# stsievert/pytorch-ps-mpi

Measured on AMD Instinct MI355X. Metric: samples/sec (node) ResNet-50 async PS at 1/2/4/8 MI355X; grad bytes/step, higher is better.
Workload: dtype bf16

## Files before the change

hipps/csrc/bindings.cpp:

```cpp
#include <torch/extension.h>
#include <vector>

namespace hipps {
void aggregate(const std::vector<at::Tensor>& slots, at::Tensor acc, double gscale, bool accumulate, bool acquire);
void copy_acquire(at::Tensor src, at::Tensor dst);
void convert(at::Tensor src, at::Tensor dst, double scale);
void gather_flat(const std::vector<at::Tensor>& srcs, at::Tensor table, at::Tensor dst, double scale);
void transpose_cast(at::Tensor src, at::Tensor dst, at::Tensor tiles);
void sgd_step(const std::vector<at::Tensor>& grads, double gscale, at::Tensor p, c10::optional<at::Tensor> buf,
              c10::optional<at::Tensor> pub, bool zero_src, double lr, double wd, double momentum, double dampening,
              bool nesterov, bool first, c10::optional<at::Tensor> mask, c10::optional<at::Tensor> csteps,
              double lookahead);
void adam_step(const std::vector<at::Tensor>& grads, double gscale, at::Tensor p, at::Tensor exp_avg,
               at::Tensor exp_avg_sq, c10::optional<at::Tensor> max_exp_avg_sq, c10::optional<at::Tensor> pub,
               bool zero_src, double lr, double beta1, double beta2, double eps, double wd, int64_t step,
               bool amsgrad, bool torch_mode, c10::optional<at::Tensor> mask, c10::optional<at::Tensor> csteps);
void q8_encode(at::Tensor x, c10::optional<at::Tensor> resid, at::Tensor q, at::Tensor scales, bool stochastic,
               int64_t seed);
void q8_aggregate(const std::vector<at::Tensor>& qs, const std::vector<at::Tensor>& ss, at::Tensor acc, double gscale,
                  bool accumulate, bool acquire);
void topk_encode(at::Tensor g, c10::optional<at::Tensor> resid, int64_t k, at::Tensor idx, at::Tensor val,
                 at::Tensor workspace);
int64_t topk_workspace_bytes(int64_t n, int64_t k);
void topk_accumulate(at::Tensor idx, at::Tensor val, at::Tensor acc, double gscale, bool acquire);
// ... 23 lines not shown
void bn_backward_partials(at::Tensor part, int64_t nrb, at::Tensor dy, at::Tensor x, int64_t mask_mode,
                          at::Tensor weight, at::Tensor mean, at::Tensor invstd, at::Tensor scale, at::Tensor shift,
                          at::Tensor dx, c10::optional<at::Tensor> dres, at::Tensor dweight, at::Tensor dbias, int64_t C,
                          c10::optional<at::Tensor> mask_in, int64_t unr);
int64_t conv1x1_mtiles(int64_t M);
void conv1x1_forward(at::Tensor x, at::Tensor w, at::Tensor y, c10::optional<at::Tensor> part, int64_t Hi,
                     int64_t Wi, int64_t stride, c10::optional<at::Tensor> add, c10::optional<at::Tensor> add_mask,
                     c10::optional<at::Tensor> bn_x, c10::optional<at::Tensor> bn_bits,
                     c10::optional<at::Tensor> bn_mean, c10::optional<at::Tensor> bn_invstd,
                     c10::optional<at::Tensor> bn_scale, c10::optional<at::Tensor> bn_shift,
                     c10::optional<at::Tensor> pro_scale, c10::optional<at::Tensor> pro_shift);
void bn_dual_forward(at::Tensor part3, int64_t nrb3, at::Tensor partd, int64_t nrbd, at::Tensor x3, at::Tensor xd,
                     at::Tensor z, at::Tensor mask, at::Tensor w3, at::Tensor b3, at::Tensor rm3, at::Tensor rv3,
                     at::Tensor mean3, at::Tensor invstd3, at::Tensor scale3, at::Tensor shift3, at::Tensor wd,
                     at::Tensor bd, at::Tensor rmd, at::Tensor rvd, at::Tensor meand, at::Tensor invstdd,
                     at::Tensor scaled, at::Tensor shiftd, int64_t C, double eps3, double mom3, double epsd,
                     double momd);
void bn_dual_backward(c10::optional<at::Tensor> part3, int64_t nrb3, at::Tensor dz, at::Tensor x3, at::Tensor xd,
                      at::Tensor mask, at::Tensor w3, at::Tensor mean3, at::Tensor invstd3, at::Tensor wd,
                      at::Tensor meand, at::Tensor invstdd, at::Tensor dx3, at::Tensor dxd, at::Tensor dw3,
                      at::Tensor db3, at::Tensor dwd, at::Tensor dbd, int64_t C, int64_t unr);
at::Tensor gemm2_dgrad_s2(at::Tensor dy, at::Tensor wf, at::Tensor dx, int64_t bm, int64_t bn,
                          c10::optional<at::Tensor> bn_x, c10::optional<at::Tensor> bn_bits,
                          c10::optional<at::Tensor> bn_mean, c10::optional<at::Tensor> bn_invstd,
                          c10::optional<at::Tensor> bn_scale, c10::optional<at::Tensor> bn_shift);
int64_t gemm2_mtiles(int64_t M, int64_t N, int64_t K, int64_t bm);
void gemm2_conv(at::Tensor x, at::Tensor w, at::Tensor y, c10::optional<at::Tensor> part,
                c10::optional<at::Tensor> add, c10::optional<at::Tensor> add_mask, int64_t Hi, int64_t Wi,
                int64_t stride, int64_t KH, int64_t KW, int64_t pad, int64_t bm, int64_t bn,
                c10::optional<at::Tensor> bn_x, c10::optional<at::Tensor> bn_bits, c10::optional<at::Tensor> bn_mean,
                c10::optional<at::Tensor> bn_invstd, c10::optional<at::Tensor> bn_scale,
                c10::optional<at::Tensor> bn_shift, int64_t stages, bool add_s2,
                c10::optional<at::Tensor> pro_scale, c10::optional<at::Tensor> pro_shift,
                c10::optional<at::Tensor> bias, c10::optional<at::Tensor> gelu_pre, int64_t gelu);
void gemm2_wgrad(at::Tensor dy, at::Tensor x, at::Tensor dw, int64_t KH, int64_t KW, int64_t stride, int64_t pad,
                 int64_t Hi, int64_t Wi, int64_t cfg, int64_t stages,
                 c10::optional<at::Tensor> pro_scale, c10::optional<at::Tensor> pro_shift, int64_t sdiv);
void maxpool3s2_forward(at::Tensor x, at::Tensor y, at::Tensor code, c10::optional<at::Tensor> scale,
                        c10::optional<at::Tensor> shift);
void bn_finalize_partials(at::Tensor part, int64_t nrb, int64_t M, at::Tensor weight, at::Tensor bias,
                          c10::optional<at::Tensor> running_mean, c10::optional<at::Tensor> running_var,
                          at::Tensor mean, at::Tensor invstd, at::Tensor scale, at::Tensor shift, int64_t C, double eps,
                          double momentum);
void maxpool3s2_backward(at::Tensor dy, at::Tensor code, at::Tensor dx);
std::vector<at::Tensor> xent_forward(at::Tensor logits, at::Tensor labels, int64_t ignore_index);
void colsum_fold(at::Tensor part, at::Tensor out);
void colsum_bf16(at::Tensor x, at::Tensor out);
std::vector<at::Tensor> attn_forward(at::Tensor q, at::Tensor k, at::Tensor v, bool causal, double scale,
                                     c10::optional<at::Tensor> kvlen);
std::vector<at::Tensor> attn_backward(at::Tensor dout, at::Tensor q, at::Tensor k, at::Tensor v, at::Tensor o,
                                      at::Tensor lse, bool causal, double scale, c10::optional<at::Tensor> kvlen,
                                      c10::optional<at::Tensor> dq_out, c10::optional<at::Tensor> dk_out,
                                      c10::optional<at::Tensor> dv_out);
void swiglu_forward(at::Tensor a, at::Tensor b, at::Tensor c);
void ln_forward(at::Tensor x, at::Tensor w, at::Tensor b, at::Tensor y, at::Tensor mean, at::Tensor rstd, double eps);
void ln_backward(at::Tensor dy, at::Tensor x, at::Tensor mean, at::Tensor rstd, at::Tensor w, at::Tensor dx,
                 at::Tensor dw, at::Tensor db, c10::optional<at::Tensor> dxsum);
void embed_forward(at::Tensor ids, c10::optional<at::Tensor> tt, at::Tensor word, at::Tensor pos, at::Tensor typ,
                   at::Tensor out);
void embed_pos_backward(at::Tensor dout, at::Tensor dpos, int64_t B, int64_t S);
void embed_seg_backward(at::Tensor dout, at::Tensor sid, at::Tensor perm, at::Tensor dtab);
void rms_forward(at::Tensor x, at::Tensor w, at::Tensor y, at::Tensor rstd, double eps, c10::optional<at::Tensor> add,
                 c10::optional<at::Tensor> xsum);
void rms_backward(at::Tensor dy, at::Tensor x, at::Tensor rstd, at::Tensor w, at::Tensor dx, at::Tensor dw,
                  c10::optional<at::Tensor> dres, c10::optional<at::Tensor> dx16);
void swiglu_backward(at::Tensor g, at::Tensor a, at::Tensor b, at::Tensor da, at::Tensor db);
void rope_apply(at::Tensor x, at::Tensor y, at::Tensor cs, at::Tensor sn, int64_t S, int64_t hd, double sign);
// ... 74 lines not shown
        py::arg("acc"), py::arg("gscale"), py::arg("acquire") = false);
  m.def("topk_q8_accumulate", &hipps::topk_q8_accumulate, "acc[idx] += gscale * deq(q)", py::arg("idx"), py::arg("q"),
        py::arg("scales"), py::arg("acc"), py::arg("gscale"), py::arg("acquire") = false);
  m.def("topk_q8_residual", &hipps::topk_q8_residual, "EF: r[idx] += v - deq(q)");
  m.def("thresh_encode", &hipps::thresh_encode, "variable-size |x|>tau sparsification, device count header");
  m.def("thresh_accumulate", &hipps::thresh_accumulate, "acc[idx[:count]] += gscale * val[:count]", py::arg("count"),
        py::arg("idx"), py::arg("val"), py::arg("acc"), py::arg("gscale"), py::arg("acquire") = false);
  m.def("copy_counted", &hipps::copy_counted, "copy a [count | idx | val] message moving only count entries");
  m.def("bn_forward_train", &hipps::bn_forward_train, "fused channels-last BN train fwd (+res) (+relu)");
  m.def("bn_apply", &hipps::bn_apply, "y = act(x*scale + shift (+res))");
  m.def("bn_backward", &hipps::bn_backward, "fused BN bwd with relu-mask recompute (+dres)");
  m.def("bn_forward_partials", &hipps::bn_forward_partials, "BN fwd finalize+apply from producer-reduced partials");
  m.def("bn_backward_partials", &hipps::bn_backward_partials, "BN bwd finalize+apply from consumer-reduced partials",
        py::arg("part"), py::arg("nrb"), py::arg("dy"), py::arg("x"), py::arg("mask_mode"), py::arg("weight"),
        py::arg("mean"), py::arg("invstd"), py::arg("scale"), py::arg("shift"), py::arg("dx"), py::arg("dres"),
        py::arg("dweight"), py::arg("dbias"), py::arg("C"), py::arg("mask_in"), py::arg("unr") = 0);
  m.def("conv1x1_mtiles", &hipps::conv1x1_mtiles);
  m.def("bn_dual_forward", &hipps::bn_dual_forward,
        "z = relu(bn3(x3) + bnd(xd)) from producer partials: two finalizes + one apply (downsample block)");
  m.def("bn_dual_backward", &hipps::bn_dual_backward,
        "backward of bn_dual_forward: dx3 + the downsample BN's reduction in one pass, then dxd",
        py::arg("part3"), py::arg("nrb3"), py::arg("dz"), py::arg("x3"), py::arg("xd"), py::arg("mask"), py::arg("w3"),
        py::arg("mean3"), py::arg("invstd3"), py::arg("wd"), py::arg("meand"), py::arg("invstdd"), py::arg("dx3"),
        py::arg("dxd"), py::arg("dw3"), py::arg("db3"), py::arg("dwd"), py::arg("dbd"), py::arg("C"),
        py::arg("unr") = 4);
  m.def("gemm2_mtiles", &hipps::gemm2_mtiles, py::arg("M"), py::arg("N"), py::arg("K"), py::arg("bm") = 0);
  m.def("gemm2_conv", &hipps::gemm2_conv, "second-generation MFMA conv GEMM (LDS-DMA staged, 256-row tiles)",
        py::arg("x"), py::arg("w"), py::arg("y"), py::arg("part") = py::none(), py::arg("add") = py::none(),
        py::arg("add_mask") = py::none(), py::arg("Hi"), py::arg("Wi"), py::arg("stride") = 1, py::arg("KH") = 1,
        py::arg("KW") = 1, py::arg("pad") = 0, py::arg("bm") = 0, py::arg("bn") = 0, py::arg("bn_x") = py::none(),
        py::arg("bn_bits") = py::none(), py::arg("bn_mean") = py::none(), py::arg("bn_invstd") = py::none(),
        py::arg("bn_scale") = py::none(), py::arg("bn_shift") = py::none(), py::arg("stages") = 2,
        py::arg("add_s2") = false, py::arg("pro_scale") = py::none(), py::arg("pro_shift") = py::none(),
        py::arg("bias") = py::none(), py::arg("gelu_pre") = py::none(), py::arg("gelu") = 0);
  m.def("gemm2_dgrad_s2", &hipps::gemm2_dgrad_s2,
        "stride-2 3x3 input gradient as four output-parity implicit GEMMs (+ BN-backward reduction)",
        py::arg("dy"), py::arg("wf"), py::arg("dx"), py::arg("bm") = 128, py::arg("bn") = 128,
        py::arg("bn_x") = py::none(), py::arg("bn_bits") = py::none(), py::arg("bn_mean") = py::none(),
        py::arg("bn_invstd") = py::none(), py::arg("bn_scale") = py::none(), py::arg("bn_shift") = py::none());
  m.def("gemm2_wgrad", &hipps::gemm2_wgrad, "conv weight gradient on the LDS-DMA MFMA core (split-M slabs)",
        py::arg("dy"), py::arg("x"), py::arg("dw"), py::arg("KH"), py::arg("KW"), py::arg("stride"), py::arg("pad"),
        py::arg("Hi"), py::arg("Wi"), py::arg("cfg") = 0, py::arg("stages") = 2, py::arg("pro_scale") = py::none(),
        py::arg("pro_shift") = py::none(), py::arg("sdiv") = 1);
  m.def("conv1x1_forward", &hipps::conv1x1_forward,
        "MFMA 1x1 conv (NHWC GEMM) with fused BN-stats epilogue and optional (+ add * mask) epilogue",
        pybind11::arg("x"), pybind11::arg("w"), pybind11::arg("y"), pybind11::arg("part"), pybind11::arg("Hi"),
        pybind11::arg("Wi"), pybind11::arg("stride"), pybind11::arg("add") = pybind11::none(),
        pybind11::arg("add_mask") = pybind11::none(), pybind11::arg("bn_x") = pybind11::none(),
        pybind11::arg("bn_bits") = pybind11::none(), pybind11::arg("bn_mean") = pybind11::none(),
        pybind11::arg("bn_invstd") = pybind11::none(), pybind11::arg("bn_scale") = pybind11::none(),
        pybind11::arg("bn_shift") = pybind11::none(), pybind11::arg("pro_scale") = pybind11::none(),
        pybind11::arg("pro_shift") = pybind11::none());
  m.def("convkxk_forward", &hipps::convkxk_forward,
        "MFMA KxK conv forward (implicit GEMM, channels-last bf16) with optional BN-statistics epilogue",
        pybind11::arg("x"), pybind11::arg("w"), pybind11::arg("y"), pybind11::arg("part") = pybind11::none(),
        pybind11::arg("stride") = 1, pybind11::arg("pad") = 1);
  m.def("stem_mtiles", &hipps::stem_mtiles, "number of BN partial-statistic columns of stem_forward");
  m.def("stem_forward", &hipps::stem_forward,
        "ResNet stem 7x7/s2/p3 3->64 conv forward on MFMA (channels-last bf16), optional BN-statistics epilogue",
        pybind11::arg("x"), pybind11::arg("w"), pybind11::arg("y"), pybind11::arg("part") = pybind11::none());
  m.def("stem_bnpool_backward", &hipps::stem_bnpool_backward,
        "backward of maxpool(relu(bn(stem(x)))): BN parameter grads + stem weight grad, no pool gradient "
        "materialised (the BN input gradient only with materialize_dy)",
        py::arg("dp"), py::arg("code"), py::arg("y"), py::arg("x"), py::arg("bn_weight"), py::arg("mean"),
        py::arg("invstd"), py::arg("scale"), py::arg("shift"), py::arg("dbn_w"), py::arg("dbn_b"), py::arg("dw"),
        py::arg("materialize_dy") = false, py::arg("quad") = true);
  m.def("stem_wgrad", &hipps::stem_wgrad, "ResNet stem 7x7/s2/p3 weight gradient on MFMA (fp32 dW, deterministic)");
// ... 82 lines not shown
```

hipps/csrc/gemm2.hip:

```cpp
#include "common.h"

#include <ATen/ATen.h>
#include <cstdlib>
#include <mutex>
#include <c10/hip/HIPStream.h>
#include <torch/extension.h>

namespace hipps {
namespace g2 {

typedef short bf16x8 __attribute__((ext_vector_type(8)));
typedef float f32x4 __attribute__((ext_vector_type(4)));
typedef float f32x16 __attribute__((ext_vector_type(16)));
typedef uint32_t u32x4 __attribute__((ext_vector_type(4)));
typedef __attribute__((address_space(3))) void lds_void;
typedef __attribute__((address_space(1))) void glb_void;

constexpr int BK = 64;

__device__ __attribute__((aligned(64))) const uint16_t kZero16[32] = {0};
__device__ __attribute__((aligned(64))) const uint8_t kOnes8[64] = {
    0xff, 0xff, 0xff, 0xff, 0xff, 0xff, 0xff, 0xff, 0xff, 0xff, 0xff, 0xff, 0xff, 0xff, 0xff, 0xff,
    0xff, 0xff, 0xff, 0xff, 0xff, 0xff, 0xff, 0xff, 0xff, 0xff, 0xff, 0xff, 0xff, 0xff, 0xff, 0xff,
    0xff, 0xff, 0xff, 0xff, 0xff, 0xff, 0xff, 0xff, 0xff, 0xff, 0xff, 0xff, 0xff, 0xff, 0xff, 0xff,
// ... 48 lines not shown
  const uint16_t* R;
  const uint8_t* RM;
  const uint16_t* bx;
  const uint8_t* bbits;
  const float *bmean, *binvstd, *bscale, *bshift;
  int M, N, K, Ho, Wo, Hi, Wi, stride, mtiles, ntiles;
  int KW, pad, Cin;
  int ldb;
  int pstride, pcol0;
  int ph, pw, Hx, Wx;
  int tdr[4], tdc[4], tko[4];
  const float *psc, *psh;
  const float* bias;
  uint16_t* Y2;
  int epf;
};

__device__ __forceinline__ uint32_t add_bf16x2(uint32_t a, uint32_t b) {
  return pack_bf16x2(__uint_as_float(a << 16) + __uint_as_float(b << 16),
                     __uint_as_float(a & 0xffff0000u) + __uint_as_float(b & 0xffff0000u));
}

__device__ __forceinline__ void glds16(const void* src, void* dst) {
  __builtin_amdgcn_global_load_lds((glb_void*)src, (lds_void*)dst, 16, 0, 0);
}

constexpr int waitcnt_vm(int n) { return (n & 15) | ((n >> 4) << 14) | (7 << 4) | (15 << 8); }
constexpr int waitcnt_lgkm(int n) { return 15 | (3 << 14) | (7 << 4) | ((n & 15) << 8); }

__host__ __device__ constexpr int khalf_swz(int row) {
  return ((0x1320 >> (4 * ((row >> 2) & 3))) & 3);
}

template <int BM, int BN, int EPI, bool TAPS, int NS>
__global__ __launch_bounds__((nthreads<BM, BN>())) void k_gemm(Args g) {
  constexpr int TM = Cfg<BM, BN>::TM, TN = Cfg<BM, BN>::TN;
  constexpr int WM = BM / TM, WN = BN / TN, NW = WM * WN, NT = 64 * NW;
  constexpr int FM = TM / 16, FN = TN / 16;
  constexpr bool KH = NS == 4;
  constexpr bool PP = NS == 5;
  constexpr bool M32 = NS == 6;
  constexpr int NSX = M32 ? 2 : NS;
  constexpr bool PAR = (EPI & kPar) != 0;
  constexpr bool PRO = (EPI & kPro) != 0;
  static_assert(!PAR || TAPS, "kPar needs the implicit-GEMM loader");
  static_assert(!PRO || NS == 2, "kPro: 2 LDS stages");
  static_assert(!PP || (BM == 256 && BN == 256), "ping-pong: 256x256 on 8 waves");
  static_assert(!M32 || (BM == 256 && BN == 256 && !PRO), "32x32x16 MFMA: the 256x256 tile");
  auto orow = [&](int m) -> int64_t {
    if constexpr (PAR) {
      const int hw = g.Ho * g.Wo;
      const int img = m / hw, rem = m - img * hw;
      const int a = rem / g.Wo, b = rem - a * g.Wo;
      return ((int64_t)img * g.Hx + 2 * a + g.ph) * g.Wx + 2 * b + g.pw;
    } else {
      return m;
    }
  };
  constexpr int STAGE = (BM + BN) * BK;
  constexpr int UNIT = (BM + BN) * 32;
  constexpr int RPI = KH ? 16 : 8;
  constexpr int AI = BM / RPI / NW;
  constexpr int BI = BN / RPI / NW;
  constexpr int EP = BN + 8;
  constexpr int NSB = (KH || PP || M32) ? 2 : NS;
  constexpr int SCR = (NSB * STAGE * 2 > BM * EP * 2 ? NSB * STAGE * 2 : BM * EP * 2);
  static_assert(AI >= 1 && BI >= 1, "tile too small for the wave count");
  static_assert(NS >= 2 && NS <= 6, "stages");
  constexpr int NG = AI + BI;
  constexpr int BIP = PP ? 2 * BI : BI;
  __shared__ __attribute__((aligned(16))) uint16_t lds[lds_bytes<BM, BN, NS>() / 2];

  const int nwg = gridDim.x, orig = blockIdx.x, xcd = orig & 7, q8 = nwg >> 3, r8 = nwg & 7;
  const int bid = (xcd < r8 ? xcd * (q8 + 1) : r8 * (q8 + 1) + (xcd - r8) * q8) + (orig >> 3);
  const int mt = bid / g.ntiles, nt = bid - mt * g.ntiles;
  const int m0 = mt * BM, n0 = nt * BN;
  const int t = threadIdx.x, lane = t & 63;
  const int w = __builtin_amdgcn_readfirstlane(t >> 6);
  const int wm = w / WN, wn = w - (w / WN) * WN;
  auto arb = [&](int i) { return PP ? (BM / 2) * wm + RPI * (i * (NW / 2) + wn) : RPI * (i * NW + w); };
  auto brb = [&](int i) { return PP ? RPI * (i * (NW / 2) + wn) : RPI * (i * NW + w); };
  const int lr = KH ? lane >> 2 : lane >> 3;
  const int lc = KH ? (lane & 3) ^ khalf_swz(lr)
                    : M32 ? (lane & 7) ^ (((lr >> 1) | ((w & 1) << 2)) & 7) : (lane & 7) ^ lr;

  const uint16_t* a_src[AI];
  int a_h[TAPS ? AI : 1], a_w[TAPS ? AI : 1];
  bool a_ok[AI];
#pragma unroll
  for (int i = 0; i < AI; ++i) {
    const int row = arb(i) + lr;
    int m = m0 + row;
    a_ok[i] = m < g.M;
    m = a_ok[i] ? m : g.M - 1;
    if constexpr (TAPS) {
      const int hw = g.Ho * g.Wo;
      const int img = m / hw, rem = m - img * hw;
      const int ho = rem / g.Wo, wo = rem - ho * g.Wo;
      a_h[i] = PAR ? ho : ho * g.stride - g.pad;
      a_w[i] = PAR ? wo : wo * g.stride - g.pad;
      a_src[i] = g.X + (int64_t)img * g.Hi * g.Wi * g.Cin + lc * 8;
    } else {
      int64_t src = m;
      if (g.stride != 1) {
        const int hw = g.Ho * g.Wo;
        const int img = m / hw, rem = m - img * hw;
        const int ho = rem / g.Wo, wo = rem - ho * g.Wo;
        src = ((int64_t)img * g.Hi + (int64_t)ho * g.stride) * g.Wi + (int64_t)wo * g.stride;
      }
      a_src[i] = g.X + src * g.K + lc * 8;
    }
  }
  const uint16_t* b_src0 = g.W + (int64_t)(n0 + brb(0) + lr) * g.ldb + lc * 8;
  auto b_src = [&](int i) { return b_src0 + (int64_t)(brb(i) - brb(0)) * g.ldb; };

  uint32_t pro_ok = 0;
  float pro_sc[PRO ? 8 : 1], pro_sh[PRO ? 8 : 1];
  auto issue_at = [&](int k0, uint16_t* base, int rowlen, bool do_b = true) {
    int bk = k0;
    if constexpr (PRO) {
      const int ch = (TAPS ? k0 - (k0 / g.Cin) * g.Cin : k0) + lc * 8;
      const float4 s0 = *reinterpret_cast<const float4*>(g.psc + ch);
      const float4 s1 = *reinterpret_cast<const float4*>(g.psc + ch + 4);
// ... 7 lines not shown
    }
    if constexpr (TAPS) {
      const int tap = k0 / g.Cin, c0 = k0 - tap * g.Cin;
      int kr, kc;
      if constexpr (PAR) {
        kr = g.tdr[tap];
        kc = g.tdc[tap];
        bk = g.tko[tap] * g.Cin + c0;
      } else {
        kr = tap / g.KW;
        kc = tap - kr * g.KW;
      }
#pragma unroll
      for (int i = 0; i < AI; ++i) {
        const int hi = a_h[i] + kr, wi = a_w[i] + kc;
        const bool ok = a_ok[i] && hi >= 0 && hi < g.Hi && wi >= 0 && wi < g.Wi;
        const uint16_t* p = ok ? a_src[i] + ((int64_t)hi * g.Wi + wi) * g.Cin + c0 : kZero16;
        glds16(p, base + arb(i) * rowlen);
        if constexpr (PRO) pro_ok |= (ok ? 1u : 0u) << i;
      }
    } else {
#pragma unroll
      for (int i = 0; i < AI; ++i) {
        glds16(a_ok[i] ? a_src[i] + k0 : kZero16, base + arb(i) * rowlen);
        if constexpr (PRO) pro_ok |= (a_ok[i] ? 1u : 0u) << i;
      }
    }
    if (do_b) {
#pragma unroll
      for (int i = 0; i < BIP; ++i) glds16(b_src(i) + bk, base + BM * rowlen + brb(i) * rowlen);
    }
  };
  auto issue = [&](int kt, int s) { issue_at(kt * BK, lds + s * STAGE, BK); };
  auto issue_unit = [&](int u) { issue_at(u * 32, lds + (u & 3) * UNIT, 32); };

  f32x4 acc[FM][FN];
#pragma unroll
  for (int i = 0; i < FM; ++i)
#pragma unroll
    for (int j = 0; j < FN; ++j) acc[i][j] = f32x4{0.f, 0.f, 0.f, 0.f};
  constexpr int FM2 = M32 ? TM / 32 : 1, FN2 = M32 ? TN / 32 : 1;
  f32x16 acc32[FM2][FN2];
  if constexpr (M32) {
#pragma unroll
    for (int i = 0; i < FM2; ++i)
#pragma unroll
      for (int j = 0; j < FN2; ++j)
#pragma unroll
        for (int r = 0; r < 16; ++r) acc32[i][j][r] = 0.f;
  }

  constexpr bool ADDE = (EPI & kAdd) != 0;
  constexpr bool S2 = (EPI & kAddS2) != 0;
  constexpr int BSTE = (EPI & kBstBits) ? 2 : (EPI & kBst) ? 1 : 0;
  constexpr bool GELUB = (EPI & kGeluB) != 0;
  constexpr bool XS = BSTE || GELUB;
  auto r_off = [&](int m, int col) -> int64_t {
    if constexpr (S2) {
      const int hw = g.Ho * g.Wo;
      const int img = m / hw, rem = m - img * hw;
      const int h = rem / g.Wo, wv = rem - h * g.Wo;
      if ((h | wv) & 1) return -1;
      const int hs = (g.Ho + 1) >> 1, ws = (g.Wo + 1) >> 1;
      return (((int64_t)img * hs + (h >> 1)) * ws + (wv >> 1)) * g.N + col;
    } else {
      return (int64_t)m * g.N + col;
// ... 69 lines not shown
          for (int j = 0; j < FN; ++j)
            acc[i][j] = __builtin_amdgcn_mfma_f32_16x16x32_bf16(a[slot][i], b[slot][j], acc[i][j], 0, 0, 0);
        __builtin_amdgcn_s_setprio(0);
      }
    };
    issue_at(0, lds, BK, g1);
    if (KT > 1) issue_at(BK, lds + STAGE, BK, g1);
    asm volatile("s_waitcnt vmcnt(0)" ::: "memory");
    __builtin_amdgcn_s_barrier();
    if (g1) __builtin_amdgcn_s_barrier();
    for (int kt = 0; kt < KT; ++kt) {
      compute(kt);
      if (!g1) {
        __builtin_amdgcn_s_barrier();
        asm volatile("" ::: "memory");
        if (kt + 2 < KT) {
          issue_at((kt + 2) * BK, lds + (kt & 1) * STAGE, BK, false);
          __builtin_amdgcn_s_waitcnt(waitcnt_vm(AI));
        } else {
          asm volatile("s_waitcnt vmcnt(0)" ::: "memory");
        }
        __builtin_amdgcn_s_barrier();
        asm volatile("" ::: "memory");
      } else {
        asm volatile("s_waitcnt vmcnt(0)" ::: "memory");
        __builtin_amdgcn_s_barrier();
        asm volatile("" ::: "memory");
        if (kt + 2 < KT) issue_at((kt + 2) * BK, lds + (kt & 1) * STAGE, BK, true);
        __builtin_amdgcn_s_barrier();
        asm volatile("" ::: "memory");
      }
    }
    if (!g1) __builtin_amdgcn_s_barrier();
  } else if constexpr (KH) {
    const int NU = g.K / 32;
    issue_unit(0);
    if (NU > 1) issue_unit(1);
    if (NU > 2) issue_unit(2);
    for (int u = 0; u < NU; ++u) {
      const int younger = (NU - 1 - u) < 2 ? (NU - 1 - u) : 2;
      if (younger == 2) __builtin_amdgcn_s_waitcnt(waitcnt_vm(2 * NG));
      else if (younger == 1) __builtin_amdgcn_s_waitcnt(waitcnt_vm(NG));
      else asm volatile("s_waitcnt vmcnt(0)" ::: "memory");
      asm volatile("s_waitcnt lgkmcnt(0)" ::: "memory");
      __builtin_amdgcn_s_barrier();
      asm volatile("" ::: "memory");
      if (u + 3 < NU) issue_unit(u + 3);
      else if (u + 1 == NU) prefetch_epi();
      const uint16_t* As = lds + (u & 3) * UNIT;
      const uint16_t* Bs = As + BM * 32;
      bf16x8 a[FM], b[FN];
      const int c = lane >> 4;
#pragma unroll
      for (int j = 0; j < FN; ++j) {
        const int row = wn * TN + j * 16 + (lane & 15);
        b[j] = *reinterpret_cast<const bf16x8*>(Bs + row * 32 + ((c ^ khalf_swz(row)) << 3));
      }
#pragma unroll
      for (int i = 0; i < FM; ++i) {
        const int row = wm * TM + i * 16 + (lane & 15);
        a[i] = *reinterpret_cast<const bf16x8*>(As + row * 32 + ((c ^ khalf_swz(row)) << 3));
      }
      __builtin_amdgcn_s_setprio(1);
#pragma unroll
      for (int i = 0; i < FM; ++i)
#pragma unroll
// ... 298 lines not shown
            bsa[2 * j] += __uint_as_float(vw[j] << 16);
            bsa[2 * j + 1] += __uint_as_float(vw[j] & 0xffff0000u);
          }
        }
      }
      *reinterpret_cast<uint4*>(g.Y + o) = v;
      if (BST) {
        u32x4 xu;
        uint32_t mbits;
        if constexpr (PF) {
          xu = px[i];
          mbits = pxm[i];
        } else {
          xu = lx[b];
          mbits = lxm[b];
        }
        const uint32_t dv[4] = {v.x, v.y, v.z, v.w};
        const uint32_t xw[4] = {xu.x, xu.y, xu.z, xu.w};
#pragma unroll
        for (int j = 0; j < 8; ++j) {
          const float d = __uint_as_float(j & 1 ? dv[j >> 1] & 0xffff0000u : dv[j >> 1] << 16);
          const float xv = __uint_as_float(j & 1 ? xw[j >> 1] & 0xffff0000u : xw[j >> 1] << 16);
          const bool on = BST == 2 ? ((mbits >> j) & 1u) != 0u : fmaf(xv, bsc[j], bsh[j]) > 0.f;
          const float dz = on ? d : 0.f;
          bsa[j] += dz;
          bsb[j] = fmaf(dz, (xv - bmu[j]) * bis[j], bsb[j]);
        }
      }
    }
  }
  }
  if (BST || GBS) {
    constexpr int RL = NT / RCH;
    static_assert(2 * RL * BN * 4 <= lds_bytes<BM, BN, NS>(), "BST scratch");
    float* red = reinterpret_cast<float*>(lds);
    __syncthreads();
#pragma unroll
    for (int j = 0; j < 8; ++j) {
      red[(t / RCH) * BN + cc + j] = bsa[j];
      red[RL * BN + (t / RCH) * BN + cc + j] = bsb[j];
    }
    __syncthreads();
    if (t < BN) {
      float sa = 0.f, sb = 0.f;
      for (int r = 0; r < RL; ++r) {
        sa += red[r * BN + t];
        sb += red[RL * BN + r * BN + t];
      }
      if constexpr (GBS) {
        g.pa[(int64_t)mt * g.N + n0 + t] = sa;
      } else {
        g.pa[(int64_t)(n0 + t) * g.pstride + g.pcol0 + mt] = sa;
        g.pb[(int64_t)(n0 + t) * g.pstride + g.pcol0 + mt] = sb;
      }
    }
  }
  if (STATS && t < BN) {
    float sa = 0.f, qa = 0.f;
#pragma unroll
    for (int i = 0; i < WM; ++i) {
      sa += st[(i * BN + t) * 2];
      qa += st[(i * BN + t) * 2 + 1];
    }
    g.pa[(int64_t)(n0 + t) * g.pstride + g.pcol0 + mt] = sa;
    g.pb[(int64_t)(n0 + t) * g.pstride + g.pcol0 + mt] = qa;
  }
}
// ... 331 lines not shown
        for (int u = 0; u < 4; ++u) {
          a[u].x += b[u].x; a[u].y += b[u].y; a[u].z += b[u].z; a[u].w += b[u].w;
        }
      }
      for (; s < s1; ++s) {
        const float4 b = *reinterpret_cast<const float4*>(base + (int64_t)s * NK);
        a[0].x += b.x; a[0].y += b.y; a[0].z += b.z; a[0].w += b.w;
      }
      float4 r;
      r.x = (a[0].x + a[1].x) + (a[2].x + a[3].x);
      r.y = (a[0].y + a[1].y) + (a[2].y + a[3].y);
      r.z = (a[0].z + a[1].z) + (a[2].z + a[3].z);
      r.w = (a[0].w + a[1].w) + (a[2].w + a[3].w);
      if (gi == 0) {
        tot = r;
      } else {
        tot.x += r.x; tot.y += r.y; tot.z += r.z; tot.w += r.w;
      }
    }
    *reinterpret_cast<float4*>(g.dw + (int64_t)n * g.K + k) = tot;
  }
}

inline void pick_tile(int64_t M, int64_t N, int64_t K, int& bm, int& bn) {
  auto blocks = [&](int a, int b) { return ((M + a - 1) / a) * (N / b); };
  if (N % 256 == 0 && ((K >= 1024 && blocks(256, 256) >= 192 && blocks(128, 128) < 1536) ||
                       (K >= 2048 && blocks(256, 256) >= 512))) {
    bm = 256; bn = 256; return;
  }
  if (N % 128 == 0) { bm = 128; bn = 128; return; }
  bm = 128; bn = 64;
}

}

int64_t gemm2_mtiles(int64_t M, int64_t N, int64_t K, int64_t bm) {
  int b = (int)bm, n = 0;
  if (b <= 0) g2::pick_tile(M, N, K, b, n);
  return (M + b - 1) / b;
}

void gemm2_conv(at::Tensor x, at::Tensor w, at::Tensor y, c10::optional<at::Tensor> part,
                c10::optional<at::Tensor> add, c10::optional<at::Tensor> add_mask, int64_t Hi, int64_t Wi,
                int64_t stride, int64_t KH, int64_t KW, int64_t pad, int64_t bm, int64_t bn,
                c10::optional<at::Tensor> bn_x, c10::optional<at::Tensor> bn_bits, c10::optional<at::Tensor> bn_mean,
                c10::optional<at::Tensor> bn_invstd, c10::optional<at::Tensor> bn_scale,
                c10::optional<at::Tensor> bn_shift, int64_t stages, bool add_s2,
                c10::optional<at::Tensor> pro_scale, c10::optional<at::Tensor> pro_shift,
                c10::optional<at::Tensor> bias, c10::optional<at::Tensor> gelu_pre, int64_t gelu) {
  TORCH_CHECK(x.is_cuda() && w.is_cuda() && y.is_cuda(), "gemm2: device tensors");
  TORCH_CHECK(stages >= 2 && stages <= 6,
              "gemm2: stages must be 2, 3, 4 (k-half units), 5 (ping-pong) or 6 (32x32x16 MFMA)");
  TORCH_CHECK(x.scalar_type() == at::kBFloat16 && w.scalar_type() == at::kBFloat16 &&
                  y.scalar_type() == at::kBFloat16, "gemm2: bf16 tensors");
  const int64_t N = w.size(0), K = w.numel() / N, Cin = K / (KH * KW);
  TORCH_CHECK(Cin * KH * KW == K && Cin % g2::BK == 0 && N % 64 == 0, "gemm2: needs Cin % 64 == 0, Cout % 64 == 0");
  const int64_t imgs = x.numel() / (Cin * Hi * Wi);
  TORCH_CHECK(imgs * Cin * Hi * Wi == x.numel(), "gemm2: x size");
  const int64_t Ho = (Hi + 2 * pad - KH) / stride + 1, Wo = (Wi + 2 * pad - KW) / stride + 1;
  const int64_t M = imgs * Ho * Wo;
  TORCH_CHECK(y.numel() == M * N, "gemm2: y size");
  TORCH_CHECK(w.is_contiguous() || w.is_contiguous(at::MemoryFormat::ChannelsLast), "gemm2: dense w");
  for (const at::Tensor* t : {&x, &w, &y})
    TORCH_CHECK(reinterpret_cast<uintptr_t>(t->data_ptr()) % 16 == 0, "gemm2: 16-byte aligned tensors");
  TORCH_CHECK(x.dim() != 4 || x.is_contiguous(at::MemoryFormat::ChannelsLast), "gemm2: channels-last x");
  TORCH_CHECK(y.dim() != 4 || y.is_contiguous(at::MemoryFormat::ChannelsLast), "gemm2: channels-last y");
  TORCH_CHECK(w.dim() != 4 || KH * KW == 1 || w.is_contiguous(at::MemoryFormat::ChannelsLast), "gemm2: channels-last w");
  TORCH_CHECK(M < (int64_t(1) << 31) && x.numel() < (int64_t(1) << 40), "gemm2: size");
  int BMv = (int)bm, BNv = (int)bn;
  if (BMv <= 0 || BNv <= 0) g2::pick_tile(M, N, K, BMv, BNv);
  TORCH_CHECK(N % BNv == 0, "gemm2: Cout must be a multiple of the block tile");
  const int64_t mtiles = (M + BMv - 1) / BMv, ntiles = N / BNv;
  TORCH_CHECK(mtiles * ntiles < (int64_t(1) << 31), "gemm2: grid");
  g2::Args a{};
  a.X = (const uint16_t*)x.data_ptr();
  a.W = (const uint16_t*)w.data_ptr();
  a.Y = (uint16_t*)y.data_ptr();
  a.M = (int)M; a.N = (int)N; a.K = (int)K; a.Ho = (int)Ho; a.Wo = (int)Wo; a.Hi = (int)Hi; a.Wi = (int)Wi;
  a.stride = (int)stride; a.mtiles = (int)mtiles; a.ntiles = (int)ntiles;
  a.KW = (int)KW; a.pad = (int)pad; a.Cin = (int)Cin;
  a.ldb = (int)K; a.pstride = (int)mtiles; a.pcol0 = 0;
  int epi = g2::kPlain;
// ... 62 lines not shown
  if (gelu_pre.has_value() && gelu_pre->defined()) {
    TORCH_CHECK(epi == g2::kPlain && !taps && (gelu == 1 || gelu == 2),
                "gemm2: the GELU epilogues run on a plain 1x1 GEMM (gelu=1 forward, 2 backward)");
    TORCH_CHECK(gelu_pre->is_cuda() && gelu_pre->scalar_type() == at::kBFloat16 && gelu_pre->numel() == M * N &&
                    gelu_pre->is_contiguous() && reinterpret_cast<uintptr_t>(gelu_pre->data_ptr()) % 16 == 0,
                "gemm2: gelu_pre must be a 16-byte aligned contiguous bf16 tensor shaped like y");
    if (gelu == 1) {
      a.Y2 = (uint16_t*)gelu_pre->data_ptr();
      epi |= g2::kGelu;
    } else {
      TORCH_CHECK(!(bias.has_value() && bias->defined()), "gemm2: the GELU backward epilogue takes no bias");
      a.bx = (const uint16_t*)gelu_pre->data_ptr();
      epi |= g2::kGeluB;
      if (a.pa != nullptr) epi |= g2::kGeluBS;
    }
  } else {
    TORCH_CHECK(gelu == 0, "gemm2: gelu needs gelu_pre");
  }
  if (bias.has_value() && bias->defined()) {
    TORCH_CHECK((epi == g2::kPlain || epi == g2::kAdd || epi == g2::kGelu) && !taps,
                "gemm2: the bias epilogue runs on a 1x1 GEMM, alone or with a plain add (a residual)");
    TORCH_CHECK(bias->is_cuda() && bias->scalar_type() == at::kFloat && bias->is_contiguous() && bias->numel() == N,
                "gemm2: bias must be f32 [Cout]");
    a.bias = bias->data_ptr<float>();
    epi |= g2::kBias;
  }
  static const int epf_env = [] {
    const char* e = std::getenv("HIPPS_G2_EPF");
    return e ? std::atoi(e) : 1;
  }();
  a.epf = epf_env;
  auto stream = c10::hip::getCurrentHIPStream();
  const int grid = (int)(mtiles * ntiles);
#define HIPPS_G2S(BMc, BNc, EPc, TPc, NSc) \
  hipLaunchKernelGGL((g2::k_gemm<BMc, BNc, EPc, TPc, NSc>), grid, (g2::nthreads<BMc, BNc>()), 0, stream, a)
#define HIPPS_G2(BMc, BNc, EPc, TPc) \
  do {                                                      \
    if (NS3) HIPPS_G2S(BMc, BNc, EPc, TPc, NS3_OF(BMc, BNc)); \
    else if (NS4) HIPPS_G2S(BMc, BNc, EPc, TPc, 4);          \
    else if (NS5) HIPPS_G2S(BMc, BNc, EPc, TPc, NS5_OF(BMc, BNc)); \
    else if (NS6) HIPPS_G2S(BMc, BNc, EPc, TPc, NS6_OF(BMc, BNc)); \
    else HIPPS_G2S(BMc, BNc, EPc, TPc, 2);                   \
  } while (0)
#define HIPPS_G2_E(BMc, BNc)                                                                        \
  do {                                                                                              \
    if (taps) {                                                                                     \
      switch (epi) {                                                                                \
        case g2::kStats | g2::kPro: HIPPS_G2S(BMc, BNc, (g2::kStats | g2::kPro), true, 2); break;    \
        case g2::kStats: HIPPS_G2(BMc, BNc, g2::kStats, true); break;                               \
        case g2::kBst: HIPPS_G2(BMc, BNc, g2::kBst, true); break;                                   \
        case g2::kBstBits: HIPPS_G2(BMc, BNc, g2::kBstBits, true); break;                           \
        default: HIPPS_G2(BMc, BNc, g2::kPlain, true); break;                                       \
      }                                                                                             \
    } else {                                                                                        \
      switch (epi) {                                                                                \
        case g2::kStats | g2::kPro: HIPPS_G2S(BMc, BNc, (g2::kStats | g2::kPro), false, 2); break;   \
        case g2::kStats: HIPPS_G2(BMc, BNc, g2::kStats, false); break;                              \
        case g2::kAdd: HIPPS_G2(BMc, BNc, g2::kAdd, false); break;                                  \
        case g2::kBias: HIPPS_G2(BMc, BNc, g2::kBias, false); break;                                \
        case g2::kBias | g2::kAdd: HIPPS_G2(BMc, BNc, (g2::kBias | g2::kAdd), false); break;        \
        case g2::kGelu: HIPPS_G2(BMc, BNc, g2::kGelu, false); break;                                \
        case g2::kBias | g2::kGelu: HIPPS_G2(BMc, BNc, (g2::kBias | g2::kGelu), false); break;      \
        case g2::kGeluB: HIPPS_G2(BMc, BNc, g2::kGeluB, false); break;                              \
        case g2::kGeluB | g2::kGeluBS: HIPPS_G2(BMc, BNc, (g2::kGeluB | g2::kGeluBS), false); break;  \
        case g2::kBst: HIPPS_G2(BMc, BNc, g2::kBst, false); break;                                  \
        case g2::kBst | g2::kAdd: HIPPS_G2(BMc, BNc, (g2::kBst | g2::kAdd), false); break;          \
// ... 284 lines not shown
```

Before: 12120.

## Stage 3x3 conv A operand as one LDS strip per tile for reuse across taps

Adds a strip-staging path to the implicit-GEMM 3x3 stride-1 conv kernel. Each tile loads a contiguous strip of input rows (tile rows plus a halo of two image rows) into LDS once. All nine taps then read shifted windows of that strip, with per-row boundary masks zeroing out-of-image taps, instead of re-gathering A for every tap. It is enabled by default for Cin 64/128 layers whose LDS fits under a threshold. The cost is a larger LDS footprint, which may lower occupancy, plus extra masking work.

Result: no change. 12200, median of 6 (+0.7%).

```diff
diff --git a/hipps/csrc/bindings.cpp b/hipps/csrc/bindings.cpp
--- a/hipps/csrc/bindings.cpp
+++ b/hipps/csrc/bindings.cpp
@@ -79,7 +79,9 @@
                 c10::optional<at::Tensor> bn_invstd, c10::optional<at::Tensor> bn_scale,
                 c10::optional<at::Tensor> bn_shift, int64_t stages, bool add_s2,
                 c10::optional<at::Tensor> pro_scale, c10::optional<at::Tensor> pro_shift,
-                c10::optional<at::Tensor> bias, c10::optional<at::Tensor> gelu_pre, int64_t gelu);
+                c10::optional<at::Tensor> bias, c10::optional<at::Tensor> gelu_pre, int64_t gelu, int64_t strip);
+bool gemm2_strip_applies(int64_t Cin, int64_t Hi, int64_t Wi, int64_t KH, int64_t KW, int64_t stride, int64_t pad,
+                         int64_t bm, int64_t bn, int64_t stages, bool prologue);
 void gemm2_wgrad(at::Tensor dy, at::Tensor x, at::Tensor dw, int64_t KH, int64_t KW, int64_t stride, int64_t pad,
                  int64_t Hi, int64_t Wi, int64_t cfg, int64_t stages,
                  c10::optional<at::Tensor> pro_scale, c10::optional<at::Tensor> pro_shift, int64_t sdiv);
@@ -220,7 +222,11 @@
         py::arg("bn_bits") = py::none(), py::arg("bn_mean") = py::none(), py::arg("bn_invstd") = py::none(),
         py::arg("bn_scale") = py::none(), py::arg("bn_shift") = py::none(), py::arg("stages") = 2,
         py::arg("add_s2") = false, py::arg("pro_scale") = py::none(), py::arg("pro_shift") = py::none(),
-        py::arg("bias") = py::none(), py::arg("gelu_pre") = py::none(), py::arg("gelu") = 0);
+        py::arg("bias") = py::none(), py::arg("gelu_pre") = py::none(), py::arg("gelu") = 0, py::arg("strip") = -1);
+  m.def("gemm2_strip_applies", &hipps::gemm2_strip_applies,
+        "whether gemm2_conv can stage this convolution's A operand as one strip per tile (strip=1)",
+        py::arg("Cin"), py::arg("Hi"), py::arg("Wi"), py::arg("KH"), py::arg("KW"), py::arg("stride"), py::arg("pad"),
+        py::arg("bm"), py::arg("bn"), py::arg("stages") = 2, py::arg("prologue") = false);
   m.def("gemm2_dgrad_s2", &hipps::gemm2_dgrad_s2,
         "stride-2 3x3 input gradient as four output-parity implicit GEMMs (+ BN-backward reduction)",
         py::arg("dy"), py::arg("wf"), py::arg("dx"), py::arg("bm") = 128, py::arg("bn") = 128,
diff --git a/hipps/csrc/gemm2.hip b/hipps/csrc/gemm2.hip
--- a/hipps/csrc/gemm2.hip
+++ b/hipps/csrc/gemm2.hip
@@ -104,8 +104,9 @@
   return ((0x1320 >> (4 * ((row >> 2) & 3))) & 3);
 }
 
-template <int BM, int BN, int EPI, bool TAPS, int NS>
+template <int BM, int BN, int EPI, bool TAPS, int NS, int SLDS = 0>
 __global__ __launch_bounds__((nthreads<BM, BN>())) void k_gemm(Args g) {
+  constexpr bool STRIP = SLDS > 0;
   constexpr int TM = Cfg<BM, BN>::TM, TN = Cfg<BM, BN>::TN;
   constexpr int WM = BM / TM, WN = BN / TN, NW = WM * WN, NT = 64 * NW;
   constexpr int FM = TM / 16, FN = TN / 16;
@@ -119,6 +120,7 @@
   static_assert(!PRO || NS == 2, "kPro: 2 LDS stages");
   static_assert(!PP || (BM == 256 && BN == 256), "ping-pong: 256x256 on 8 waves");
   static_assert(!M32 || (BM == 256 && BN == 256 && !PRO), "32x32x16 MFMA: the 256x256 tile");
+  static_assert(!STRIP || (TAPS && NS == 2 && !PAR && !PRO), "strip staging: the plain 3x3 loader, 2 stages");
   auto orow = [&](int m) -> int64_t {
     if constexpr (PAR) {
       const int hw = g.Ho * g.Wo;
@@ -136,12 +138,12 @@
   constexpr int BI = BN / RPI / NW;
   constexpr int EP = BN + 8;
   constexpr int NSB = (KH || PP || M32) ? 2 : NS;
-  constexpr int SCR = (NSB * STAGE * 2 > BM * EP * 2 ? NSB * STAGE * 2 : BM * EP * 2);
+  constexpr int SCR = STRIP ? BM * EP * 2 : (NSB * STAGE * 2 > BM * EP * 2 ? NSB * STAGE * 2 : BM * EP * 2);
   static_assert(AI >= 1 && BI >= 1, "tile too small for the wave count");
   static_assert(NS >= 2 && NS <= 6, "stages");
   constexpr int NG = AI + BI;
   constexpr int BIP = PP ? 2 * BI : BI;
-  __shared__ __attribute__((aligned(16))) uint16_t lds[lds_bytes<BM, BN, NS>() / 2];
+  __shared__ __attribute__((aligned(16))) uint16_t lds[(STRIP ? SLDS : lds_bytes<BM, BN, NS>()) / 2];
 
   const int nwg = gridDim.x, orig = blockIdx.x, xcd = orig & 7, q8 = nwg >> 3, r8 = nwg & 7;
   const int bid = (xcd < r8 ? xcd * (q8 + 1) : r8 * (q8 + 1) + (xcd - r8) * q8) + (orig >> 3);
@@ -160,7 +162,7 @@
   int a_h[TAPS ? AI : 1], a_w[TAPS ? AI : 1];
   bool a_ok[AI];
 #pragma unroll
-  for (int i = 0; i < AI; ++i) {
+  for (int i = 0; i < (STRIP ? 0 : AI); ++i) {
     const int row = arb(i) + lr;
     int m = m0 + row;
     a_ok[i] = m < g.M;
@@ -234,6 +236,14 @@
     }
   };
   auto issue = [&](int kt, int s) { issue_at(kt * BK, lds + s * STAGE, BK); };
+  const int srp = (BM + 2 * g.Wi + 2 + 7) & ~7;
+  auto issue_strip = [&](int j0, int j1, int sl) {
+    for (int j = j0 + w; j < j1; j += NW) {
+      const int p = m0 - g.Wi - 1 + 8 * j + lr;
+      const bool ok = p >= 0 && p < g.M;
+      glds16(ok ? g.X + (int64_t)p * g.Cin + sl * BK + lc * 8 : kZero16, lds + (sl * srp + 8 * j) * BK);
+    }
+  };
   auto issue_unit = [&](int u) { issue_at(u * 32, lds + (u & 3) * UNIT, 32); };
 
   f32x4 acc[FM][FN];
@@ -369,6 +379,82 @@
       }
     }
     if (!g1) __builtin_amdgcn_s_barrier();
+  } else if constexpr (STRIP) {
+    const int KT = g.K / BK, CS = g.Cin / BK, NJ = srp >> 3;
+    uint16_t* const Bst = lds + CS * srp * BK;
+    auto issue_b = [&](int kt, int s) {
+#pragma unroll
+      for (int i = 0; i < BI; ++i) glds16(b_src(i) + kt * BK, Bst + s * BN * BK + brb(i) * BK);
+    };
+    uint32_t amask[FM];
+#pragma unroll
+    for (int i = 0; i < FM; ++i) {
+      const int m = m0 + wm * TM + i * 16 + (lane & 15);
+      const int hw = g.Hi * g.Wi;
+      const int rem = m - (m / hw) * hw;
+      const int ho = rem / g.Wi, wo = rem - ho * g.Wi;
+      const uint32_t cm = (wo > 0 ? 1u : 0u) | 2u | (wo + 1 < g.Wi ? 4u : 0u);
+      const uint32_t rm = (ho > 0 ? cm : 0u) | (cm << 3) | (ho + 1 < g.Hi ? cm << 6 : 0u);
+      amask[i] = m < g.M ? rm : 0u;
+    }
+    issue_strip(0, BM / 8, 0);
+    issue_b(0, 0);
+    int cur = 0, tap = 0, sl = 0, soff = 0, kc = 0;
+    for (int kt = 0; kt < KT; ++kt) {
+      asm volatile("s_waitcnt vmcnt(0) lgkmcnt(0)" ::: "memory");
+      __builtin_amdgcn_s_barrier();
+      asm volatile("" ::: "memory");
+      if (kt == 0) {
+        issue_strip(BM / 8, NJ, 0);
+        for (int s = 1; s < CS; ++s) issue_strip(0, NJ, s);
+      }
+      if (kt + 1 < KT) issue_b(kt + 1, cur ^ 1);
+      else prefetch_epi();
+      const uint16_t* As = lds + sl * srp * BK;
+      const uint16_t* Bs = Bst + cur * BN * BK;
+      cur ^= 1;
+      constexpr int KS = BK / 32;
+      bf16x8 a[KS][FM], b[KS][FN];
+#pragma unroll
+      for (int ks = 0; ks < KS; ++ks) {
+        const int c = ks * 4 + (lane >> 4);
+#pragma unroll
+        for (int j = 0; j < FN; ++j) {
+          const int row = wn * TN + j * 16 + (lane & 15);
+          b[ks][j] = *reinterpret_cast<const bf16x8*>(Bs + row * BK + ((c ^ (row & 7)) << 3));
+        }
+#pragma unroll
+        for (int i = 0; i < FM; ++i) {
+          const int row = soff + wm * TM + i * 16 + (lane & 15);
+          a[ks][i] = *reinterpret_cast<const bf16x8*>(As + row * BK + ((c ^ (row & 7)) << 3));
+        }
+      }
+#pragma unroll
+      for (int ks = 0; ks < KS; ++ks) {
+        if (ks == 0 && FM + FN <= 15) __builtin_amdgcn_s_waitcnt(waitcnt_lgkm(FM + FN));
+#pragma unroll
+        for (int i = 0; i < FM; ++i) {
+          const bool out = ((amask[i] >> tap) & 1u) == 0u;
+          if (__builtin_amdgcn_ballot_w64(out) != 0) a[ks][i] = out ? bf16x8{0, 0, 0, 0, 0, 0, 0, 0} : a[ks][i];
+        }
+        __builtin_amdgcn_s_setprio(1);
+#pragma unroll
+        for (int i = 0; i < FM; ++i)
+#pragma unroll
+          for (int j = 0; j < FN; ++j)
+            acc[i][j] = __builtin_amdgcn_mfma_f32_16x16x32_bf16(a[ks][i], b[ks][j], acc[i][j], 0, 0, 0);
+        __builtin_amdgcn_s_setprio(0);
+      }
+      if (++sl == CS) {
+        sl = 0;
+        ++tap;
+        ++soff;
+        if (++kc == 3) {
+          kc = 0;
+          soff += g.Wi - 3;
+        }
+      }
+    }
   } else if constexpr (KH) {
     const int NU = g.K / 32;
     issue_unit(0);
@@ -733,7 +819,7 @@
   }
   if (BST || GBS) {
     constexpr int RL = NT / RCH;
-    static_assert(2 * RL * BN * 4 <= lds_bytes<BM, BN, NS>(), "BST scratch");
+    static_assert(2 * RL * BN * 4 <= (STRIP ? BM * EP * 2 : lds_bytes<BM, BN, NS>()), "BST scratch");
     float* red = reinterpret_cast<float*>(lds);
     __syncthreads();
 #pragma unroll
@@ -1131,6 +1217,34 @@
   bm = 128; bn = 64;
 }
 
+constexpr int kStripLds3 = 52 * 1024, kStripLds2 = 80 * 1024, kStripLdsMax = 160 * 1024;
+inline int64_t strip_rows(int64_t bm, int64_t Wi) { return (bm + 2 * Wi + 2 + 7) / 8 * 8; }
+inline int64_t strip_lds(int64_t Cin, int64_t Wi, int64_t bm, int64_t bn) {
+  const int64_t k = (Cin / BK) * strip_rows(bm, Wi) * BK * 2 + 2 * bn * BK * 2;
+  const int64_t e = bm * (bn + 8) * 2 + 2 * 2 * 2 * bn * 4;
+  return k > e ? k : e;
+}
+
+template <int BM, int BN, int EPI>
+void launch_strip(const Args& a, int grid, hipStream_t stream) {
+  const int64_t lds = strip_lds(a.Cin, a.Wi, BM, BN);
+  if (BN == 64 && lds <= kStripLds3)
+    hipLaunchKernelGGL((k_gemm<BM, BN, EPI, true, 2, (BN == 64 ? kStripLds3 : kStripLds2)>), grid, (nthreads<BM, BN>()), 0,
+                       stream, a);
+  else if (lds <= kStripLds2)
+    hipLaunchKernelGGL((k_gemm<BM, BN, EPI, true, 2, kStripLds2>), grid, (nthreads<BM, BN>()), 0, stream, a);
+  else
+    hipLaunchKernelGGL((k_gemm<BM, BN, EPI, true, 2, kStripLdsMax>), grid, (nthreads<BM, BN>()), 0, stream, a);
+}
+
+}
+
+bool gemm2_strip_applies(int64_t Cin, int64_t Hi, int64_t Wi, int64_t KH, int64_t KW, int64_t stride, int64_t pad,
+                         int64_t bm, int64_t bn, int64_t stages, bool prologue) {
+  if (KH != 3 || KW != 3 || stride != 1 || pad != 1 || stages != 2 || prologue) return false;
+  if (Hi < 1 || Wi < 1 || (Cin != 64 && Cin != 128)) return false;
+  if (bm != 128 || (bn != 64 && bn != 128)) return false;
+  return g2::strip_lds(Cin, Wi, bm, bn) <= g2::kStripLdsMax;
 }
 
 int64_t gemm2_mtiles(int64_t M, int64_t N, int64_t K, int64_t bm) {
@@ -1146,7 +1260,7 @@
                 c10::optional<at::Tensor> bn_invstd, c10::optional<at::Tensor> bn_scale,
                 c10::optional<at::Tensor> bn_shift, int64_t stages, bool add_s2,
                 c10::optional<at::Tensor> pro_scale, c10::optional<at::Tensor> pro_shift,
-                c10::optional<at::Tensor> bias, c10::optional<at::Tensor> gelu_pre, int64_t gelu) {
+                c10::optional<at::Tensor> bias, c10::optional<at::Tensor> gelu_pre, int64_t gelu, int64_t strip) {
   TORCH_CHECK(x.is_cuda() && w.is_cuda() && y.is_cuda(), "gemm2: device tensors");
   TORCH_CHECK(stages >= 2 && stages <= 6,
               "gemm2: stages must be 2, 3, 4 (k-half units), 5 (ping-pong) or 6 (32x32x16 MFMA)");
@@ -1275,6 +1389,28 @@
   a.epf = epf_env;
   auto stream = c10::hip::getCurrentHIPStream();
   const int grid = (int)(mtiles * ntiles);
+  static const int strip_env = [] {
+    const char* e = std::getenv("HIPPS_G2_STRIP");
+    return e ? std::atoi(e) : 1;
+  }();
+  TORCH_CHECK(strip >= -1 && strip <= 1, "gemm2: strip must be -1 (auto), 0 or 1");
+  const bool strip_ok = gemm2_strip_applies(Cin, Hi, Wi, KH, KW, stride, pad, BMv, BNv, stages, (epi & g2::kPro) != 0) &&
+                        (epi & ~(g2::kStats | g2::kBst | g2::kBstBits)) == 0 && M + 4 * Wi + 1024 < (int64_t(1) << 31);
+  TORCH_CHECK(strip != 1 || strip_ok, "gemm2: strip staging does not apply to this call");
+  if (strip == 1 || (strip == -1 && strip_env != 0 && strip_ok && !(Cin == 128 && BNv == 64) &&
+                     g2::strip_lds(Cin, Wi, BMv, BNv) <= g2::kStripLds2)) {
+#define HIPPS_G2_STRIP_E(BMc, BNc)                                                               \
+  switch (epi) {                                                                                 \
+    case g2::kStats: g2::launch_strip<BMc, BNc, g2::kStats>(a, grid, stream); break;             \
+    case g2::kBst: g2::launch_strip<BMc, BNc, g2::kBst>(a, grid, stream); break;                 \
+    case g2::kBstBits: g2::launch_strip<BMc, BNc, g2::kBstBits>(a, grid, stream); break;         \
+    default: g2::launch_strip<BMc, BNc, g2::kPlain>(a, grid, stream); break;                     \
+  }
+    if (BNv == 64) HIPPS_G2_STRIP_E(128, 64)
+    else HIPPS_G2_STRIP_E(128, 128)
+#undef HIPPS_G2_STRIP_E
+    return;
+  }
 #define HIPPS_G2S(BMc, BNc, EPc, TPc, NSc) \
   hipLaunchKernelGGL((g2::k_gemm<BMc, BNc, EPc, TPc, NSc>), grid, (g2::nthreads<BMc, BNc>()), 0, stream, a)
 #define HIPPS_G2(BMc, BNc, EPc, TPc) \
```
